# wkentaro/morefusion

Hardware: AMD Instinct MI355X
Metric: objects/sec (32^3 voxelize+3D-CNN+ICC refine) (higher is better)
Workload: dtype f32; 1 GPU; 1 scene(s) x 8 objects per GPU: singleview_3d Model.predict (ResNet18+PSPNet, 32^3 voxelize, occupancy 3D-CNN, heads; B=8) -> ICC joint refine 100 iters (BASELINE configs[1]+configs[2]); random weights, ICC starts from synthetic perturbed-GT poses; ICC(k) on a second HIP stream, event-ordered after network(k), beside network(k+1); objects_per_gpu=8, icc_iters=100, parallelism=scene-sharded x1, pose all_gather, stream_priority=none, backbone_memory_format=contiguous

## Files before the change

morefusion_amd/csrc/gemm_bf16.hip:

```cpp
#include <cstdlib>

#include "mf_common.h"

#include "gemm_bf16_nt.h"
#include "gemm_bf16_tn.h"
#include "gemm_bf16_aux.h"
#include "gemm_bf16_narrow.h"

namespace {

struct Knobs { int nt_big, nt_splitk, tn_pp, nt_half_max, pp_dbg; };
Knobs read_knobs() {
  auto num = [](const char *name, int unset) { const char *e = getenv(name); return e ? atoi(e) : unset; };
  Knobs k = {num("MF_NT_BIG", -1), num("MF_NT_SPLITK", 0), num("MF_TN_PP", 1), num("MF_NT_HALF_MAX", 255), 0};
#ifdef MF_PP_ABLATE
  k.pp_dbg = num("MF_PP_DBG", 0);
#endif
  return k;
}

constexpr int64_t kAnyWs = INT64_MAX;
struct NtShape { int mode; int64_t M; int N, K, groups; bool table; int64_t dgrad_rows; bool may_split; int64_t ws_bytes; };
struct NtPlan { int tile, S, dbg; };

NtPlan nt_plan(const NtShape &p, const Knobs &k) {
  const int64_t full = ((p.M + 127) / 128) * ((p.N + kBN - 1) / kBN) * p.groups;
  const int64_t big = ((p.M + kBigM - 1) / kBigM) * ((p.N + kBigN - 1) / kBigN) * p.groups;
  const bool dgrad = p.mode == kConvDgrad, can_big = !p.table && !(dgrad && (p.dgrad_rows & (kBigM - 1)));
  int S = 1;
  if (p.may_split && p.ws_bytes > 0 && can_big && p.N >= 192 && p.N % 8 == 0 && k.nt_big != 0) {
    const int T = (p.K + kBK - 1) / kBK;
    if (k.nt_splitk > 0) S = k.nt_splitk <= T ? k.nt_splitk : 1;
    else if (big >= 16 && big < 160)
      for (S = (int)(256 / big); S > 1 && T / S < 16;) --S;
    if (S > 1 && p.ws_bytes < S * p.M * p.N * 4) S = 1;
  }
  bool use_big = (big >= 224 && p.N >= 160 && can_big) || S > 1;
  if (k.nt_big == 2)
    use_big = can_big;
  else if (k.nt_big >= 0)
    use_big = use_big && k.nt_big == 1;
  if (use_big) return {kBigM, S, k.pp_dbg};
  const bool half = full <= k.nt_half_max && !dgrad;
  return {half ? 64 : 128, S, 0};
}

int64_t nt_workspace_bytes(int mode, int64_t M, int N, int K) {
  const NtPlan p = nt_plan({mode, M, N, K, 1, false, 0, true, kAnyWs}, read_knobs());
  return p.S > 1 ? p.S * M * N * 4 : 0;
}

int wgrad_split_model(int64_t tiles, int64_t ktiles, int64_t slab_bytes, int slots) {
  if (tiles <= 0 || ktiles <= 0) return 1;
  const double per_slab = slab_bytes / 3.0e6 > 0.05 ? slab_bytes / 3.0e6 : 0.05;
  int best = 1;
  double best_cost = 1e30;
  for (int S = 1; S <= 512; ++S) {
    if (S > 1 && ktiles / S < 8) break;
    const int64_t rounds = (tiles * S + slots - 1) / slots;
    const double cost = (double)rounds * (double)((ktiles + S - 1) / S + 8) + (S > 1 ? S * per_slab : 0.0);
    if (cost < best_cost) { best_cost = cost; best = S; }
  }
  return best;
}

struct TnShape { int Ni, Nj, ldc; int64_t ktiles; int groups; bool ranges, conv; int split; };
enum { kFinishNone = 0, kFinishPlain = 1, kFinishDeep = 2, kFinishConv = 3 };
struct TnPlan { bool pp; int split, finish; };

TnPlan tn_plan(const TnShape &p, const Knobs &k) {
  const int64_t tiles_pp = (int64_t)((p.Ni + 255) / 256) * ((p.Nj + 255) / 256) * p.groups;
  bool pp = k.tn_pp != 0 && k.nt_big != 0 && !p.ranges;
  if (pp && k.nt_big != 2)
    pp = p.Ni >= 192 && p.Nj >= 192 && p.ktiles >= 48 * (tiles_pp >= 256 ? 1 : (256 + tiles_pp - 1) / tiles_pp);
  const int64_t tiles = (int64_t)((p.Ni + 127) / 128) * ((p.Nj + 127) / 128) * p.groups, slab_bytes = 4ll * p.Ni * p.Nj * p.groups;
  const int split = p.split > 0 ? p.split : pp ? wgrad_split_model(tiles_pp, 2 * p.ktiles, slab_bytes, 256)
                                               : wgrad_split_model(tiles, p.ktiles, slab_bytes, 512);
  const int64_t per_slab = (int64_t)p.Ni * p.ldc * p.groups;
  int finish = split >= 32 && per_slab <= (1 << 16) ? kFinishDeep : kFinishPlain;
  if (p.conv && per_slab >= (1 << 20)) finish = kFinishConv;
  if (!p.conv && split == 1) finish = kFinishNone;
  return {pp, split, finish};
}

int g_nt_last_tile = 0;

template <int MODE, int MI>
int launch_nt_tile(const NtArgs &a, hipStream_t stream) {
  if (int e = mf::allow_big_lds((const void *)k_gemm_nt_bf16<MODE, MI>, nt_lds<MI>())) return e;
  const int64_t grid = (int64_t)((a.M + 64 * MI - 1) / (64 * MI)) * ((a.N + kBN - 1) / kBN) * a.groups;
  hipLaunchKernelGGL((k_gemm_nt_bf16<MODE, MI>), dim3((unsigned)grid), dim3(256), nt_lds<MI>(), stream, a);
  return 0;
}
template <int MODE>
int launch_nt(const NtArgs &a, const NtPlan &p, hipStream_t stream, const char *what) {
  g_nt_last_tile = p.tile;
  if (p.tile == kBigM) {
    const int64_t big = (int64_t)((a.M + kBigM - 1) / kBigM) * ((a.N + kBigN - 1) / kBigN) * a.groups;
    if (int e = mf::allow_big_lds((const void *)k_gemm_nt_bf16_pp<MODE>, nt_pp_lds())) return e;
    hipLaunchKernelGGL((k_gemm_nt_bf16_pp<MODE>), dim3((unsigned)(big * a.S)), dim3(512), nt_pp_lds(), stream, a);
    const dim3 finish((unsigned)(((int64_t)a.M * (a.N / 8) + 255) / 256));
    if (a.S > 1 && nt_split(MODE))
      hipLaunchKernelGGL(k_splitk_finish_conv2, finish, dim3(256), 0, stream, a);
    else if (a.S > 1)
      hipLaunchKernelGGL(k_splitk_finish, finish, dim3(256), 0, stream, (const float *)a.slab, a.bias, a.out,
                         (int64_t)a.M, a.N, a.S, a.ldo, a.relu, a.out_f32);
  } else if (int e = p.tile == 64 ? launch_nt_tile<MODE, 1>(a, stream) : launch_nt_tile<MODE, 2>(a, stream))
    return e;
  return mf::check_launch(what);
}

template <bool CONV>
int launch_tn(const TnArgs &a, const TnPlan &p, hipStream_t stream) {
  if (p.pp) {
    if (int e = mf::allow_big_lds((const void *)k_gemm_tn_bf16_pp<CONV>, 5 * kPpOp)) return e;
    const int64_t grid = (int64_t)((a.Ni + 255) / 256) * ((a.Nj + 255) / 256) * a.groups * a.S;
    hipLaunchKernelGGL(k_gemm_tn_bf16_pp<CONV>, dim3((unsigned)grid), dim3(512), 5 * kPpOp, stream, a);
    return 0;
  }
  if (int e = mf::allow_big_lds((const void *)k_gemm_tn_bf16<CONV>, kTnLds)) return e;
  const int64_t grid = (int64_t)((a.Ni + 127) / 128) * ((a.Nj + 127) / 128) * a.groups * a.S;
  hipLaunchKernelGGL(k_gemm_tn_bf16<CONV>, dim3((unsigned)grid), dim3(256), kTnLds, stream, a);
  return 0;
}

void launch_wgrad_finish(int finish, const TnArgs &a, float *dW, int w_cin, int keep, hipStream_t stream) {
  const int taps = a.conv ? a.ks * a.ks * a.ks : 0, cin = a.conv ? a.Cin : 0;
  const int64_t per_group = (int64_t)a.Ni * a.ldc, per_slab = per_group * a.groups;
  const int64_t pitch = a.conv ? (int64_t)w_cin * taps : a.ldc;
  if (finish == kFinishConv)
    hipLaunchKernelGGL(k_wgrad_finish_conv, dim3((keep + kPackTile - 1) / kPackTile, a.Ni), dim3(256), 0, stream,
                       (const float *)a.out, dW, per_slab, a.S, a.Cin, taps, w_cin, keep);
  else if (finish == kFinishDeep)
    hipLaunchKernelGGL(k_wgrad_finish_deep, dim3((unsigned)((per_slab + 3) / 4)), dim3(256), 0, stream,
                       (const float *)a.out, dW, per_slab, a.Nj, a.ldc, a.S, cin, a.c_gs, per_group, pitch, taps, keep);
  else if (finish == kFinishPlain)
    hipLaunchKernelGGL(k_wgrad_finish, dim3((unsigned)((per_slab + 255) / 256)), dim3(256), 0, stream,
                       (const float *)a.out, dW, per_slab, a.Nj, a.ldc, a.S, cin, a.c_gs, per_group, pitch, taps, keep);
}

constexpr int64_t kMaxBf16Elems = 1ll << 30;
int bad(const char *msg) {
  mf::set_last_error(hipErrorInvalidValue, msg);
  return -(int)hipErrorInvalidValue;
}

int ilog2_exact(int x) {
  int l = 0;
  while ((1 << l) < x) ++l;
  return (1 << l) == x ? l : -1;
}

struct Geom { int Do, olog, taps; };
int conv_geom(int B, int Cin, int Cout, int D, int ks, int stride, int pad, int dil, Geom *g) {
  const int span = dil * (ks - 1) + 1;
  if ((ks != 3 && ks != 4) || (stride != 1 && stride != 2) || dil < 1 || pad < 0 || D + 2 * pad < span)
    return bad("conv3d (bf16): kernel 3 or 4, stride 1 or 2");
  g->Do = (D + 2 * pad - span) / stride + 1;
  g->olog = ilog2_exact(g->Do);
  g->taps = ks * ks * ks;
  if (g->olog < 1 || Cin % 8 || Cout % 8 || (int64_t)B * D * D * D * Cin >= kMaxBf16Elems ||
      (int64_t)B * g->Do * g->Do * g->Do * Cout >= kMaxBf16Elems || (int64_t)Cout * g->taps * Cin >= kMaxBf16Elems)
    return bad("conv3d (bf16): output size a power of two, Cin % 8 == 0, Cout % 8 == 0, tensors < 2^30 elements (2^31 bytes)");
  return 0;
}

int conv2_geom(int B, int Cin, int Cout, int D, int ks, int stride, int pad, int dil, Geom *g) {
  const int span = dil * (ks - 1) + 1;
  if ((ks != 1 && ks != 3) || (stride != 1 && stride != 2) || dil < 1 || dil > 4 || pad < 0 || D + 2 * pad < span)
    return bad("conv2d_split: kernel 1 or 3, stride 1 or 2, dilation 1 .. 4");
  g->Do = (D + 2 * pad - span) / stride + 1;
  g->olog = ilog2_exact(g->Do);
  g->taps = ks * ks;
  if (g->olog < 0 || Cin % 8 || Cout % 8 || (int64_t)B * D * D * 2 * Cin >= kMaxBf16Elems ||
      (int64_t)B * g->Do * g->Do >= (1ll << 31) || (int64_t)Cout * g->taps * 3 * Cin >= kMaxBf16Elems)
    return bad("conv2d_split: output side a power of two, Cin % 8 == 0, Cout % 8 == 0, operands < 2^30 elements");
  return 0;
}

int split_out_check(const char *what, const float *bias, float *out32, int ldo32, void *outs, int ldos, int los, int N,
                    const float *res = nullptr, int ldr = 0) {
  if ((!out32 && !outs) || N % 8 || (out32 && (ldo32 < N || ldo32 % 8)) ||
      (outs && (ldos < N || ldos % 8 || los < N || los % 8 || ldos < los + N)) || (res && (ldr < N || ldr % 8)))
    return bad(what);
  if (((uintptr_t)bias | (uintptr_t)out32 | (uintptr_t)outs | (uintptr_t)res) & 15) return bad(what);
  return 0;
}

NtArgs nt_operands(const void *A, int lda, int64_t a_gs, const void *W, int ldw, int64_t w_gs, const float *bias,
                   int64_t b_gs, int64_t M, int N, int K, int groups, const int32_t *tile_group = nullptr) {
  NtArgs a = {};
  a.A = (const uint16_t *)A; a.W = (const uint16_t *)W; a.bias = bias;
  a.a_gs = a_gs; a.w_gs = w_gs; a.b_gs = b_gs;
  a.M = (int)M; a.N = N; a.K = K; a.lda = lda; a.ldw = ldw; a.groups = groups;
  a.tile_group = tile_group;
  return a;
}
void nt_conv_geom(NtArgs &a, int B, int D, const Geom &g, int Cin, int Cout, int ks, int stride, int pad, int dil) {
  a.B = B; a.D = D; a.Do = g.Do; a.olog = g.olog; a.Cin = Cin; a.Cout = Cout;
  a.ks = ks; a.stride = stride; a.pad = pad; a.dil = dil;
}
void nt_plain_out(NtArgs &a, void *out, int64_t o_gs, int ldo, int relu, int out_f32, int accumulate, const NtPlan &p,
                  void *ws = nullptr) {
  a.out = out; a.o_gs = o_gs; a.ldo = ldo; a.relu = relu; a.out_f32 = out_f32; a.accumulate = accumulate;
  a.S = p.S; a.slab = p.S > 1 ? (float *)ws : nullptr; a.dbg = p.dbg;
}
template <int MODE>
int launch_nt_split(NtArgs a, int xc, int act, float *out32, int ldo32, void *outs, int ldos, int los, void *ws,
                    int64_t ws_bytes, mfStream_t stream, const char *what, const float *res = nullptr, int ldr = 0,
                    const float *slope = nullptr) {
  const NtPlan p = nt_plan({MODE, a.M, a.N, a.K, 1, false, 0, true, ws ? ws_bytes : 0}, read_knobs());
  a.xc = xc; a.act = act; a.ldo32 = ldo32; a.ldos = ldos; a.los = los; a.out32 = out32; a.outs = (uint16_t *)outs;
  a.res = res; a.ldr = ldr; a.slope = slope;
  a.S = p.S; a.slab = p.S > 1 ? (float *)ws : nullptr; a.dbg = p.dbg;
  return launch_nt<MODE>(a, p, (hipStream_t)stream, what);
}

}

extern "C" int mf_gemm_bf16_nt_plan(int32_t mode, int64_t M, int32_t N, int32_t K, int32_t groups, int32_t table,
                                    int64_t dgrad_rows, int32_t may_split, int32_t have_ws, int32_t *tile, int32_t *S) {
  if (mode < kRows || mode > kRowsS || M <= 0 || N <= 0 || K <= 0 || groups <= 0 || !tile || !S)
    return bad("gemm_bf16_nt_plan: a mode 0 .. 5, a problem, somewhere to answer");
  const NtShape s = {mode, M, N, K, groups, table != 0, dgrad_rows, may_split != 0, have_ws ? kAnyWs : 0};
  const NtPlan p = nt_plan(s, read_knobs());
  *tile = p.tile; *S = p.S;
  return 0;
}

extern "C" int mf_gemm_bf16_tn_plan(int32_t Ni, int32_t Nj, int32_t ldc, int64_t rows, int32_t groups, int32_t ranges,
                                    int32_t conv, int32_t split, int32_t *form, int32_t *default_split, int32_t *finish) {
  if (Ni <= 0 || Nj <= 0 || ldc < Nj || rows < 0 || groups <= 0 || !form || !default_split || !finish)
    return bad("gemm_bf16_tn_plan: a problem with ldc >= Nj, somewhere to answer");
  const Knobs k = read_knobs();
  TnShape s = {Ni, Nj, ldc, (rows + 63) / 64, groups, ranges != 0, conv != 0, 0};
  *default_split = s.split = tn_plan(s, k).split;
  if (split > 0) s.split = split;
  const TnPlan p = tn_plan(s, k);
  *form = p.pp ? 256 : 128; *finish = p.finish;
  return 0;
}

extern "C" int mf_gemm_bf16_last_tile(void) { return g_nt_last_tile; }

extern "C" int mf_cast_rows_bf16(const float *src, int64_t src_ld, void *dst, int64_t dst_ld, int64_t rows,
                                 int32_t cols, mfStream_t stream_) {
  hipStream_t stream = (hipStream_t)stream_;
  if (rows <= 0) return 0;
  if (dst_ld % 8 || cols > dst_ld || src_ld < cols || ((uintptr_t)dst & 15)) return bad("cast_rows_bf16: dst_ld % 8 == 0, cols <= dst_ld");
  const int64_t n = rows * (dst_ld / 8);
  hipLaunchKernelGGL(k_cast_rows_bf16, dim3((unsigned)((n + 255) / 256)), dim3(256), 0, stream, src, src_ld,
                     (uint16_t *)dst, dst_ld, rows, cols);
  return mf::check_launch("mf_cast_rows_bf16");
}

extern "C" int mf_relu_mask_bf16(const void *y, const void *dy, const float *dy32, void *dz, int64_t n,
                                 mfStream_t stream_) {
  hipStream_t stream = (hipStream_t)stream_;
  if (n <= 0) return 0;
// ... 333 lines not shown
```

morefusion_amd/csrc/gemm_bf16_nt.h:

```cpp
#pragma once
#include "mf_common.h"

namespace {

using mf::mf_f32x16;

constexpr int kBN = 128, kBK = 64;
constexpr int kPitch = 144;
template <int MI> constexpr int nt_buf_bytes() { return (64 * MI + kBN) * kPitch; }
template <int MI> constexpr int nt_lds() {
  return 2 * nt_buf_bytes<MI>() > 64 * MI * (kBN + 4) * 4 ? 2 * nt_buf_bytes<MI>() : 64 * MI * (kBN + 4) * 4;
}

enum { kRows = 0, kConvFwd = 1, kConvDgrad = 2, kConv2Fwd = 3, kConvFwdS = 4, kRowsS = 5 };
constexpr bool nt_conv3(int mode) { return mode == kConvFwd || mode == kConvFwdS; }
constexpr bool nt_rows(int mode) { return mode == kRows || mode == kRowsS; }
constexpr bool nt_split(int mode) { return mode == kConv2Fwd || mode == kConvFwdS || mode == kRowsS; }

struct NtArgs {
  const uint16_t *A;
  const uint16_t *W;
  const float *bias;
  void *out;
  int64_t a_gs, w_gs, b_gs, o_gs;
  int M, N, K, lda, ldw, ldo, groups;
  int relu, out_f32, accumulate;
  const int32_t *tile_group;
  int B, D, Do, olog, Cin, Cout, ks, stride, pad, dil;
  int S;
  float *slab;
  int xc, act, ldr, ldo32, ldos, los;
  const float *res, *slope;
  float *out32;
  uint16_t *outs;
  int dbg;
};

__device__ __forceinline__ void conv2_store8(const NtArgs &a, int64_t m, int n, float *v) {
  if (a.bias) {
    const float4 b0 = *reinterpret_cast<const float4 *>(a.bias + n), b1 = *reinterpret_cast<const float4 *>(a.bias + n + 4);
    v[0] += b0.x; v[1] += b0.y; v[2] += b0.z; v[3] += b0.w; v[4] += b1.x; v[5] += b1.y; v[6] += b1.z; v[7] += b1.w;
  }
  if (a.res) {
    const float *r = a.res + m * a.ldr + n;
    const float4 r0 = *reinterpret_cast<const float4 *>(r), r1 = *reinterpret_cast<const float4 *>(r + 4);
    v[0] += r0.x; v[1] += r0.y; v[2] += r0.z; v[3] += r0.w; v[4] += r1.x; v[5] += r1.y; v[6] += r1.z; v[7] += r1.w;
  }
  if (a.act) {
    const float s = a.act == 2 ? *a.slope : 0.0f;
#pragma unroll
    for (int j = 0; j < 8; ++j) v[j] = v[j] > 0.0f ? v[j] : s * v[j];
  }
  if (a.out32) {
    float4 *o = reinterpret_cast<float4 *>(a.out32 + m * a.ldo32 + n);
    o[0] = make_float4(v[0], v[1], v[2], v[3]);
    o[1] = make_float4(v[4], v[5], v[6], v[7]);
  }
  if (a.outs) {
    uint32_t h[8], l[8];
#pragma unroll
    for (int j = 0; j < 8; ++j) {
      h[j] = mf::bf16_bits(v[j]);
      l[j] = mf::bf16_bits(v[j] - mf::bf16_lo(h[j]));
    }
    uint16_t *o = a.outs + m * a.ldos + n;
    *reinterpret_cast<uint4 *>(o) = make_uint4(h[0] | h[1] << 16, h[2] | h[3] << 16, h[4] | h[5] << 16, h[6] | h[7] << 16);
    *reinterpret_cast<uint4 *>(o + a.los) =
        make_uint4(l[0] | l[1] << 16, l[2] | l[3] << 16, l[4] | l[5] << 16, l[6] | l[7] << 16);
  }
}

template <int MODE, int MI>
__global__ __launch_bounds__(256, 2) void k_gemm_nt_bf16(NtArgs a) {
  MF_DYN_LDS(unsigned char, s_raw);
  constexpr int kBM = 64 * MI, kBuf = nt_buf_bytes<MI>();
  const int tiles_m = (a.M + kBM - 1) / kBM, tiles_n = (a.N + kBN - 1) / kBN;
  const int per_group = tiles_m * tiles_n;
  const int G = gridDim.x;
  int L = blockIdx.x;
  if ((G & 7) == 0) L = (blockIdx.x & 7) * (G >> 3) + (blockIdx.x >> 3);
  const int grp = L / per_group;
  const int rem = L - grp * per_group;
  const int m0 = (rem / tiles_n) * kBM, n0 = (rem % tiles_n) * kBN;
  const int T = (a.K + kBK - 1) / kBK;

  const int tid = threadIdx.x, wave = tid >> 6, lane = tid & 63;
  const int wm = wave & 1, wn = wave >> 1;
  const int lrow = lane & 31, lhalf = lane >> 5;
  const int chunk = tid & 7, r0 = tid >> 3;

  const int Do = a.Do, dol = a.olog;
  const uint16_t *A = a.A + grp * a.a_gs;
  const uint16_t *W = a.W + grp * a.w_gs;
  if (MODE == kRows && a.tile_group) {
    const int g = a.tile_group[m0 >> 6];
    if (g < 0) return;
    W += (int64_t)g * a.w_gs;
  }
  int cls = 0;
  if (MODE == kConvDgrad) {
    cls = (m0 >> (3 * dol)) & 7;
    W += (int64_t)cls * a.N * a.ldw;
  }
  int base[2 * MI], mask[2 * MI];
#pragma unroll
  for (int i = 0; i < 2 * MI; ++i) {
    const int m = m0 + r0 + 32 * i;
    const bool row_ok = m < a.M;
    const int mm = row_ok ? m : 0;
    int mk = row_ok ? 1 << 12 : 0;
    if (nt_rows(MODE)) {
      base[i] = mm * a.lda;
    } else if (MODE == kConv2Fwd) {
      const int b = mm >> (2 * dol), o = mm & ((1 << (2 * dol)) - 1);
      const int y0 = a.stride * (o >> dol) - a.pad, x0 = a.stride * (o & (Do - 1)) - a.pad;
      base[i] = ((b * a.D + y0) * a.D + x0) * a.xc;
#pragma unroll
      for (int k = 0; k < 4; ++k) {
        mk |= ((unsigned)(y0 + a.dil * k) < (unsigned)a.D ? 1 : 0) << k;
        mk |= ((unsigned)(x0 + a.dil * k) < (unsigned)a.D ? 1 : 0) << (4 + k);
      }
    } else if (nt_conv3(MODE)) {
      const int b = mm >> (3 * dol), o = mm & ((1 << (3 * dol)) - 1);
      const int ox = o >> (2 * dol), oy = (o >> dol) & (Do - 1), oz = o & (Do - 1);
      const int x0 = a.stride * ox - a.pad, y0 = a.stride * oy - a.pad, z0 = a.stride * oz - a.pad;
      base[i] = (((b * a.D + x0) * a.D + y0) * a.D + z0) * (MODE == kConvFwdS ? a.xc : a.Cin);
#pragma unroll
      for (int k = 0; k < 4; ++k) {
        mk |= ((unsigned)(x0 + a.dil * k) < (unsigned)a.D ? 1 : 0) << k;
        mk |= ((unsigned)(y0 + a.dil * k) < (unsigned)a.D ? 1 : 0) << (4 + k);
        mk |= ((unsigned)(z0 + a.dil * k) < (unsigned)a.D ? 1 : 0) << (8 + k);
      }
    } else {
      const int h = mm & ((1 << (3 * dol)) - 1), b = mm >> (3 * dol + 3);
      const int hx = h >> (2 * dol), hy = (h >> dol) & (Do - 1), hz = h & (Do - 1);
      const int ux = hx + (cls & 1), uy = hy + ((cls >> 1) & 1), uz = hz + ((cls >> 2) & 1);
      base[i] = (((b * Do + ux) * Do + uy) * Do + uz) * a.Cout;
#pragma unroll
      for (int s = 0; s < 2; ++s) {
        mk |= ((unsigned)(ux - s) < (unsigned)Do ? 1 : 0) << s;
        mk |= ((unsigned)(uy - s) < (unsigned)Do ? 1 : 0) << (4 + s);
        mk |= ((unsigned)(uz - s) < (unsigned)Do ? 1 : 0) << (8 + s);
      }
    }
    mask[i] = mk;
  }
  uint32_t wrow[4];
#pragma unroll
  for (int i = 0; i < 4; ++i) {
    const int n = n0 + r0 + 32 * i;
    wrow[i] = 2u * (uint32_t)((int64_t)(n < a.N ? n : 0) * a.ldw);
  }

  mf_f32x16 acc[MI][2];
#pragma unroll
  for (int i = 0; i < MI; ++i)
#pragma unroll
    for (int j = 0; j < 2; ++j)
#pragma unroll
      for (int e = 0; e < 16; ++e) acc[i][j][e] = 0.0f;

  uint4 ra0P, ra1P, ra2P = make_uint4(0u, 0u, 0u, 0u), ra3P = ra2P, rb0P, rb1P, rb2P, rb3P;
  int kg = 8 * chunk, tc = 0, tx = 0, ty = 0, tz = 0;
  if (nt_conv3(MODE)) {
    const int tap = kg / a.Cin;
    tc = kg - tap * a.Cin;
    const int kxy = tap / a.ks;
    tz = tap - kxy * a.ks; tx = kxy / a.ks; ty = kxy - tx * a.ks;
  } else if (MODE == kConv2Fwd) {
    const int tap = kg / a.Cin;
    tc = kg - tap * a.Cin;
    tx = tap / a.ks; ty = tap - tx * a.ks;
  } else if (MODE == kConvDgrad) {
    tx = kg / a.Cout;
    tc = kg - tx * a.Cout;
  }
  const mf::BufRsrc Ars = mf::make_rsrc(A), Wrs = mf::make_rsrc(W);
#define MF_NT_LOAD_A(S, i_, reg_)                                                                     \
  reg_ = mf::buf_load16(Ars, (mask[i_] & bits_) == bits_ ? 2u * (uint32_t)(base[i_] + off_) : mf::kBufMasked);
#define MF_NT_LOAD_B(S, i_, reg_) reg_ = mf::buf_load16(Wrs, wrow[i_] + kofs_);
#define MF_NT_FETCH(S)                                                                                \
  {                                                                                                   \
    const bool kin_ = kg + 8 <= a.K;                                                                  \
    const uint32_t kofs_ = kin_ ? 2u * (uint32_t)kg : 0u;                                             \
    int off_ = MODE == kRowsS && kg >= a.xc ? kg - a.xc : kg, bits_ = 1 << 12;                        \
    if (nt_conv3(MODE)) {                                                                             \
      off_ = ((tx * a.D + ty) * a.D + tz) * a.dil * (MODE == kConvFwdS ? a.xc : a.Cin) +              \
             (MODE == kConvFwdS && tc >= a.xc ? tc - a.xc : tc);                                      \
      bits_ = tx < a.ks ? (1 << tx) | (16 << ty) | (256 << tz) | (1 << 12) : 1 << 13;                 \
    } else if (MODE == kConv2Fwd) {                                                                   \
      off_ = (tx * a.D + ty) * a.dil * a.xc + (tc >= a.xc ? tc - a.xc : tc);                          \
      bits_ = tx < a.ks ? (1 << tx) | (16 << ty) | (1 << 12) : 1 << 13;                               \
    } else if (MODE == kConvDgrad) {                                                                  \
      const int sx = tx & 1, sy = (tx >> 1) & 1, sz = tx >> 2;                                        \
      off_ = tc - ((sx * Do + sy) * Do + sz) * a.Cout;                                                \
      bits_ = (1 << sx) | (16 << sy) | (256 << sz) | (1 << 12);                                       \
    }                                                                                                 \
    if (!kin_) bits_ = 1 << 13;                                              \
    MF_NT_LOAD_A(S, 0, ra0##S) MF_NT_LOAD_A(S, 1, ra1##S)                                             \
    if constexpr (MI == 2) { MF_NT_LOAD_A(S, 2 * MI - 2, ra2##S) MF_NT_LOAD_A(S, 2 * MI - 1, ra3##S) } \
    MF_NT_LOAD_B(S, 0, rb0##S) MF_NT_LOAD_B(S, 1, rb1##S) MF_NT_LOAD_B(S, 2, rb2##S) MF_NT_LOAD_B(S, 3, rb3##S) \
    kg += kBK;                                                                                        \
    if (nt_conv3(MODE)) {                                                                             \
      tc += kBK;                                                                                      \
      while (tc >= a.Cin) {                                                                           \
        tc -= a.Cin;                                                                                  \
        if (++tz == a.ks) { tz = 0; if (++ty == a.ks) { ty = 0; ++tx; } }                             \
      }                                                                                               \
    } else if (MODE == kConv2Fwd) {                                                                   \
      tc += kBK;                                                                                      \
      while (tc >= a.Cin) {                                                                           \
        tc -= a.Cin;                                                                                  \
        if (++ty == a.ks) { ty = 0; ++tx; }                                                           \
      }                                                                                               \
    } else if (MODE == kConvDgrad) {                                                                  \
      tc += kBK;                                                                                      \
      while (tc >= a.Cout) { tc -= a.Cout; ++tx; }                                                    \
    }                                                                                                 \
  }
#define MF_NT_STASH(S, buf_)                                                                          \
  {                                                                                                   \
    MF_HOLD(ra0##S); MF_HOLD(ra1##S); MF_HOLD(rb0##S); MF_HOLD(rb1##S); MF_HOLD(rb2##S); MF_HOLD(rb3##S); \
    if constexpr (MI == 2) { MF_HOLD(ra2##S); MF_HOLD(ra3##S); }                                      \
    unsigned char *As_ = s_raw + (buf_) * kBuf + r0 * kPitch + 16 * chunk;                            \
    unsigned char *Bs_ = As_ + kBM * kPitch;                                                          \
    *reinterpret_cast<uint4 *>(As_) = ra0##S; *reinterpret_cast<uint4 *>(As_ + 32 * kPitch) = ra1##S; \
    if constexpr (MI == 2) {                                                                          \
      *reinterpret_cast<uint4 *>(As_ + 64 * kPitch) = ra2##S; *reinterpret_cast<uint4 *>(As_ + 96 * kPitch) = ra3##S; \
    }                                                                                                 \
    *reinterpret_cast<uint4 *>(Bs_) = rb0##S; *reinterpret_cast<uint4 *>(Bs_ + 32 * kPitch) = rb1##S; \
    *reinterpret_cast<uint4 *>(Bs_ + 64 * kPitch) = rb2##S; *reinterpret_cast<uint4 *>(Bs_ + 96 * kPitch) = rb3##S; \
  }
#ifndef MF_NT_PIPE
#define MF_NT_PIPE 1
#endif
#define MF_NT_FRAGS(set_, s_, NJ_)                                                                    \
  {                                                                                                   \
    fa[set_][0] = *reinterpret_cast<const uint4 *>(As + 32 * (s_));                                   \
    if constexpr (MI == 2) fa[set_][1] = *reinterpret_cast<const uint4 *>(As + 32 * kPitch + 32 * (s_)); \
    fb[set_][0] = *reinterpret_cast<const uint4 *>(Bs + 32 * (s_));                                   \
    if constexpr (NJ_ == 2) fb[set_][1] = *reinterpret_cast<const uint4 *>(Bs + 32 * kPitch + 32 * (s_)); \
  }
#define MF_NT_COMPUTE(buf_, NJ_)                                                                      \
  {                                                                                                   \
    asm volatile("" ::: "memory");                                                                    \
    __builtin_amdgcn_sched_barrier(0);                                                                \
    const unsigned char *As = s_raw + (buf_) * kBuf + (wm * 32 * MI + lrow) * kPitch + 16 * lhalf;    \
    const unsigned char *Bs = s_raw + (buf_) * kBuf + (kBM + wn * 64 + lrow) * kPitch + 16 * lhalf;   \
    if constexpr (MF_NT_PIPE) {                                                                       \
      uint4 fa[2][2], fb[2][2];                                                                       \
      MF_NT_FRAGS(0, 0, NJ_)                                                                          \
      __builtin_amdgcn_sched_group_barrier(0x100, MI + NJ_, 0);                                       \
      _Pragma("unroll") for (int s = 0; s < 4; ++s) {                                                 \
        const int c = s & 1;                                                                          \
        if (s < 3) MF_NT_FRAGS(c ^ 1, s + 1, NJ_)                                                     \
        _Pragma("unroll") for (int mi = 0; mi < MI; ++mi) {                                           \
          acc[mi][0] = mf::mfma_bf16_32x32x16(fa[c][mi], fb[c][0], acc[mi][0]);                       \
          if constexpr (NJ_ == 2) acc[mi][1] = mf::mfma_bf16_32x32x16(fa[c][mi], fb[c][1], acc[mi][1]); \
        }                                                                                             \
        if (s < 3) __builtin_amdgcn_sched_group_barrier(0x100, MI + NJ_, 0);                          \
        __builtin_amdgcn_sched_group_barrier(0x008, MI * NJ_, 0);                                     \
      }                                                                                               \
    } else {                                                                                          \
      _Pragma("unroll") for (int s = 0; s < 4; ++s) {                                                 \
        const uint4 a0 = *reinterpret_cast<const uint4 *>(As + 32 * s);                               \
        const uint4 b0 = *reinterpret_cast<const uint4 *>(Bs + 32 * s);                               \
        acc[0][0] = mf::mfma_bf16_32x32x16(a0, b0, acc[0][0]);                                        \
        if constexpr (NJ_ == 2) {                                                                     \
          const uint4 b1 = *reinterpret_cast<const uint4 *>(Bs + 32 * kPitch + 32 * s);               \
          acc[0][1] = mf::mfma_bf16_32x32x16(a0, b1, acc[0][1]);                                      \
          if constexpr (MI == 2) {                                                                    \
            const uint4 a1 = *reinterpret_cast<const uint4 *>(As + 32 * kPitch + 32 * s);             \
            acc[MI - 1][0] = mf::mfma_bf16_32x32x16(a1, b0, acc[MI - 1][0]);                          \
            acc[MI - 1][1] = mf::mfma_bf16_32x32x16(a1, b1, acc[MI - 1][1]);                          \
          }                                                                                           \
        } else if constexpr (MI == 2) {                                                               \
          const uint4 a1 = *reinterpret_cast<const uint4 *>(As + 32 * kPitch + 32 * s);               \
          acc[MI - 1][0] = mf::mfma_bf16_32x32x16(a1, b0, acc[MI - 1][0]);                            \
        }                                                                                             \
      }                                                                                               \
    }                                                                                                 \
    __builtin_amdgcn_sched_barrier(0);                                                                \
  }
  const int ncols = a.N - (n0 + wn * 64);
  MF_NT_FETCH(P);
  MF_NT_STASH(P, 0);
  __syncthreads();
  for (int t = 0; t < T; ++t) {
    MF_NT_FETCH(P);
    if (ncols > 32) MF_NT_COMPUTE(t & 1, 2) else if (ncols > 0) MF_NT_COMPUTE(t & 1, 1)
    MF_NT_STASH(P, (t + 1) & 1);
    __syncthreads();
  }
#undef MF_NT_FRAGS
#undef MF_NT_COMPUTE
#undef MF_NT_STASH
#undef MF_NT_FETCH
#undef MF_NT_LOAD_B
#undef MF_NT_LOAD_A

  constexpr int kEp = kBN + 4;
  float *s_out = reinterpret_cast<float *>(s_raw);
  const float *bias = a.bias && !nt_split(MODE) ? a.bias + grp * a.b_gs : nullptr;
#pragma unroll
  for (int mi = 0; mi < MI; ++mi)
#pragma unroll
    for (int ni = 0; ni < 2; ++ni) {
      const int nl = wn * 64 + ni * 32 + lrow;
      const float bn = (bias && n0 + nl < a.N) ? bias[n0 + nl] : 0.0f;
#pragma unroll
      for (int e = 0; e < 16; ++e) {
        const int ml = wm * 32 * MI + mi * 32 + (e & 3) + 8 * (e >> 2) + 4 * lhalf;
        float v = acc[mi][ni][e] + bn;
        if (a.relu && !nt_split(MODE)) v = v > 0.0f ? v : 0.0f;
        s_out[ml * kEp + nl] = v;
      }
    }
  __syncthreads();
  for (int i = tid; i < kBM * (kBN / 8); i += 256) {
    const int ml = i / (kBN / 8), c8 = i - ml * (kBN / 8);
    const int m = m0 + ml, n = n0 + 8 * c8;
    if (m >= a.M || n >= a.N) continue;
    int64_t orow = m;
    if (MODE == kConvDgrad) {
      const int h = m & ((1 << (3 * dol)) - 1), p = (m >> (3 * dol)) & 7, b = m >> (3 * dol + 3);
      const int x = 2 * (h >> (2 * dol)) + (p & 1), y = 2 * ((h >> dol) & (Do - 1)) + ((p >> 1) & 1),
                z = 2 * (h & (Do - 1)) + (p >> 2);
      orow = (((int64_t)b * a.D + x) * a.D + y) * a.D + z;
    }
    const float4 v0 = *reinterpret_cast<const float4 *>(s_out + ml * kEp + 8 * c8);
    const float4 v1 = *reinterpret_cast<const float4 *>(s_out + ml * kEp + 8 * c8 + 4);
    float v[8] = {v0.x, v0.y, v0.z, v0.w, v1.x, v1.y, v1.z, v1.w};
    if (nt_split(MODE)) {
      conv2_store8(a, m, n, v);
      continue;
    }
    const int nv = a.N - n < 8 ? a.N - n : 8;
    if (a.out_f32) {
      float *o = reinterpret_cast<float *>(a.out) + grp * a.o_gs + orow * a.ldo + n;
      if (nv == 8 && (a.ldo & 3) == 0 && ((uintptr_t)o & 15) == 0) {
        float4 *o4 = reinterpret_cast<float4 *>(o);
        if (a.accumulate) {
          const float4 p0 = o4[0], p1 = o4[1];
          v[0] += p0.x; v[1] += p0.y; v[2] += p0.z; v[3] += p0.w;
          v[4] += p1.x; v[5] += p1.y; v[6] += p1.z; v[7] += p1.w;
        }
        o4[0] = make_float4(v[0], v[1], v[2], v[3]);
        o4[1] = make_float4(v[4], v[5], v[6], v[7]);
      } else {
        for (int j = 0; j < nv; ++j) o[j] = a.accumulate ? o[j] + v[j] : v[j];
      }
    } else {
      uint16_t *o = reinterpret_cast<uint16_t *>(a.out) + grp * a.o_gs + orow * a.ldo + n;
      if (nv == 8 && (a.ldo & 7) == 0 && ((uintptr_t)o & 15) == 0) {
        *reinterpret_cast<uint4 *>(o) = make_uint4(mf::pack_bf16x2(v[0], v[1]), mf::pack_bf16x2(v[2], v[3]),
                                                   mf::pack_bf16x2(v[4], v[5]), mf::pack_bf16x2(v[6], v[7]));
      } else {
        for (int j = 0; j < nv; ++j) o[j] = (uint16_t)mf::bf16_bits(v[j]);
      }
    }
  }
}

constexpr int kBigM = 256, kBigN = 256;

constexpr int kPpOp = 256 * 128;
constexpr int kPpW0 = 3 * kPpOp;
constexpr int nt_pp_lds() { return 5 * kPpOp; }

template <int MODE>
__global__ __launch_bounds__(512, 2) void k_gemm_nt_bf16_pp(NtArgs a) {
  MF_DYN_LDS(unsigned char, s_raw);
  constexpr int kBM = kBigM, kBNb = kBigN;
  const int tiles_m = (a.M + kBM - 1) / kBM, tiles_n = (a.N + kBNb - 1) / kBNb;
  const int per_group = tiles_m * tiles_n;
  const int G = gridDim.x;
  int L = blockIdx.x;
  if ((G & 7) == 0) L = (blockIdx.x & 7) * (G >> 3) + (blockIdx.x >> 3);
  const int split = L / (per_group * a.groups);
  L -= split * per_group * a.groups;
  const int grp = L / per_group;
  const int rem = L - grp * per_group;
  const int m0 = (rem / tiles_n) * kBM, n0 = (rem % tiles_n) * kBNb;
  const int Tall = (a.K + kBK - 1) / kBK, Tper = (Tall + a.S - 1) / a.S;
  const int t0 = split * Tper;
  const int T = max(0, min(Tall, t0 + Tper) - t0);

  const int tid = threadIdx.x, lane = tid & 63;
  const int wave = mf::wave_uniform(tid >> 6);
  const int wm = wave >> 2, wn = wave & 3;
  const int lrow = lane & 31, lhalf = lane >> 5;
  const int r0 = tid >> 3;
  const int chunk = (tid & 7) ^ ((r0 >> 1) & 7);

  const int Do = a.Do, dol = a.olog;
  const uint16_t *A = a.A + grp * a.a_gs;
  const uint16_t *W = a.W + grp * a.w_gs;
  int cls = 0;
  if (MODE == kConvDgrad) {
    cls = (m0 >> (3 * dol)) & 7;
    W += (int64_t)cls * a.N * a.ldw;
  }
  int base[4], mask[4];
#pragma unroll
  for (int i = 0; i < 4; ++i) {
    const int m = m0 + r0 + 64 * i;
    const bool row_ok = m < a.M;
    const int mm = row_ok ? m : 0;
    int mk = row_ok ? 1 << 12 : 0;
    if (nt_rows(MODE)) {
      base[i] = mm * a.lda;
    } else if (MODE == kConv2Fwd) {
      const int b = mm >> (2 * dol), o = mm & ((1 << (2 * dol)) - 1);
      const int y0 = a.stride * (o >> dol) - a.pad, x0 = a.stride * (o & (Do - 1)) - a.pad;
      base[i] = ((b * a.D + y0) * a.D + x0) * a.xc;
#pragma unroll
      for (int k = 0; k < 4; ++k) {
        mk |= ((unsigned)(y0 + a.dil * k) < (unsigned)a.D ? 1 : 0) << k;
        mk |= ((unsigned)(x0 + a.dil * k) < (unsigned)a.D ? 1 : 0) << (4 + k);
      }
    } else if (nt_conv3(MODE)) {
      const int b = mm >> (3 * dol), o = mm & ((1 << (3 * dol)) - 1);
      const int ox = o >> (2 * dol), oy = (o >> dol) & (Do - 1), oz = o & (Do - 1);
      const int x0 = a.stride * ox - a.pad, y0 = a.stride * oy - a.pad, z0 = a.stride * oz - a.pad;
      base[i] = (((b * a.D + x0) * a.D + y0) * a.D + z0) * (MODE == kConvFwdS ? a.xc : a.Cin);
#pragma unroll
      for (int k = 0; k < 4; ++k) {
        mk |= ((unsigned)(x0 + a.dil * k) < (unsigned)a.D ? 1 : 0) << k;
        mk |= ((unsigned)(y0 + a.dil * k) < (unsigned)a.D ? 1 : 0) << (4 + k);
        mk |= ((unsigned)(z0 + a.dil * k) < (unsigned)a.D ? 1 : 0) << (8 + k);
      }
    } else {
      const int h = mm & ((1 << (3 * dol)) - 1), b = mm >> (3 * dol + 3);
      const int hx = h >> (2 * dol), hy = (h >> dol) & (Do - 1), hz = h & (Do - 1);
      const int ux = hx + (cls & 1), uy = hy + ((cls >> 1) & 1), uz = hz + ((cls >> 2) & 1);
      base[i] = (((b * Do + ux) * Do + uy) * Do + uz) * a.Cout;
#pragma unroll
      for (int s = 0; s < 2; ++s) {
        mk |= ((unsigned)(ux - s) < (unsigned)Do ? 1 : 0) << s;
        mk |= ((unsigned)(uy - s) < (unsigned)Do ? 1 : 0) << (4 + s);
        mk |= ((unsigned)(uz - s) < (unsigned)Do ? 1 : 0) << (8 + s);
      }
    }
    mask[i] = mk;
  }
  uint32_t wrow[4];
#pragma unroll
  for (int i = 0; i < 4; ++i) {
    const int n = n0 + r0 + 64 * i;
    wrow[i] = 2u * (uint32_t)((int64_t)(n < a.N ? n : 0) * a.ldw);
  }

  mf_f32x16 acc[4][2];
#pragma unroll
  for (int i = 0; i < 4; ++i)
#pragma unroll
    for (int j = 0; j < 2; ++j)
#pragma unroll
      for (int e = 0; e < 16; ++e) acc[i][j][e] = 0.0f;

  int kg = 8 * chunk + kBK * t0, tc = 0, tx = 0, ty = 0, tz = 0, kgw = kg;
  if (nt_conv3(MODE)) {
    const int tap = kg / a.Cin;
    tc = kg - tap * a.Cin;
    const int kxy = tap / a.ks;
    tz = tap - kxy * a.ks; tx = kxy / a.ks; ty = kxy - tx * a.ks;
  } else if (MODE == kConv2Fwd) {
    const int tap = kg / a.Cin;
    tc = kg - tap * a.Cin;
    tx = tap / a.ks; ty = tap - tx * a.ks;
  } else if (MODE == kConvDgrad) {
    tx = kg / a.Cout;
    tc = kg - tx * a.Cout;
  }
  const mf::BufRsrc Ars = mf::make_rsrc(A), Wrs = mf::make_rsrc(W);
  unsigned char *const dma0 = s_raw + 8 * wave * 128;
#define MF_PP_REQ_A(sa_, i0_, i1_)                                                                    \
  {                                                                                                   \
    const bool kin_ = kg + 8 <= a.K;                                                                  \
    int off_ = MODE == kRowsS && kg >= a.xc ? kg - a.xc : kg, bits_ = 1 << 12;                        \
    if (nt_conv3(MODE)) {                                                                             \
      off_ = ((tx * a.D + ty) * a.D + tz) * a.dil * (MODE == kConvFwdS ? a.xc : a.Cin) +              \
             (MODE == kConvFwdS && tc >= a.xc ? tc - a.xc : tc);                                      \
      bits_ = tx < a.ks ? (1 << tx) | (16 << ty) | (256 << tz) | (1 << 12) : 1 << 13;                 \
    } else if (MODE == kConv2Fwd) {                                                                   \
// ... 190 lines not shown
```

Before: 2028 objects/sec.

## Add split-K path for small-tile conv2 NT GEMMs with slab finish

Adds a split-K mode to the small/medium-tile NT GEMM kernel for 2D-conv forward shapes with narrow N (at most 128), chosen by a simple cost model that weighs per-split K work against slab traffic. Each split writes fp32 partials to a workspace slab, and the existing conv2 finish kernel reduces them and applies the epilogue. The aim is to fill the GPU when few output tiles exist but K is long, such as the backbone's low-channel convolutions. The cost is extra slab writes and reads plus one more kernel launch per GEMM.

```diff
diff --git a/morefusion_amd/csrc/gemm_bf16.hip b/morefusion_amd/csrc/gemm_bf16.hip
--- a/morefusion_amd/csrc/gemm_bf16.hip
+++ b/morefusion_amd/csrc/gemm_bf16.hip
@@ -9,10 +9,11 @@
 
 namespace {
 
-struct Knobs { int nt_big, nt_splitk, tn_pp, nt_half_max, pp_dbg; };
+struct Knobs { int nt_big, nt_splitk, tn_pp, nt_half_max, pp_dbg, nt_small_splitk; };
 Knobs read_knobs() {
   auto num = [](const char *name, int unset) { const char *e = getenv(name); return e ? atoi(e) : unset; };
-  Knobs k = {num("MF_NT_BIG", -1), num("MF_NT_SPLITK", 0), num("MF_TN_PP", 1), num("MF_NT_HALF_MAX", 255), 0};
+  Knobs k = {num("MF_NT_BIG", -1), num("MF_NT_SPLITK", 0), num("MF_TN_PP", 1), num("MF_NT_HALF_MAX", 255), 0,
+             num("MF_NT_SMALL_SPLITK", -1)};
 #ifdef MF_PP_ABLATE
   k.pp_dbg = num("MF_PP_DBG", 0);
 #endif
@@ -22,6 +23,17 @@
 constexpr int64_t kAnyWs = INT64_MAX;
 struct NtShape { int mode; int64_t M; int N, K, groups; bool table; int64_t dgrad_rows; bool may_split; int64_t ws_bytes; };
 struct NtPlan { int tile, S, dbg; };
+
+constexpr int kSmallSplitMinT = 8;
+int small_splitk_model(int64_t tiles, int T, int64_t slab_bytes) {
+  int best = 1;
+  double best_cost = 0.5 * T - 2.0;
+  for (int S = 2; tiles * S <= 256 && T / S >= kSmallSplitMinT; ++S) {
+    const double cost = 0.5 * ((T + S - 1) / S) + 3.0 + 0.35e-6 * (double)S * (double)slab_bytes;
+    if (cost < best_cost) { best_cost = cost; best = S; }
+  }
+  return best;
+}
 
 NtPlan nt_plan(const NtShape &p, const Knobs &k) {
   const int64_t full = ((p.M + 127) / 128) * ((p.N + kBN - 1) / kBN) * p.groups;
@@ -42,6 +54,14 @@
     use_big = use_big && k.nt_big == 1;
   if (use_big) return {kBigM, S, k.pp_dbg};
   const bool half = full <= k.nt_half_max && !dgrad;
+  if (S == 1 && p.mode == kConv2Fwd && p.may_split && p.ws_bytes > 0 && p.N % 8 == 0 && k.nt_small_splitk != 0) {
+    const int T = (p.K + kBK - 1) / kBK;
+    const int64_t tiles = half ? ((p.M + 63) / 64) * ((p.N + kBN - 1) / kBN) : full;
+    if (k.nt_small_splitk > 0) S = k.nt_small_splitk <= T ? k.nt_small_splitk : 1;
+    else if (p.N <= kBN)
+      S = small_splitk_model(tiles, T, p.M * p.N * 4);
+    if (S > 1 && p.ws_bytes < S * p.M * p.N * 4) S = 1;
+  }
   return {half ? 64 : 128, S, 0};
 }
 
@@ -85,11 +105,11 @@
 
 int g_nt_last_tile = 0;
 
-template <int MODE, int MI>
+template <int MODE, int MI, bool KSPLIT = false>
 int launch_nt_tile(const NtArgs &a, hipStream_t stream) {
-  if (int e = mf::allow_big_lds((const void *)k_gemm_nt_bf16<MODE, MI>, nt_lds<MI>())) return e;
-  const int64_t grid = (int64_t)((a.M + 64 * MI - 1) / (64 * MI)) * ((a.N + kBN - 1) / kBN) * a.groups;
-  hipLaunchKernelGGL((k_gemm_nt_bf16<MODE, MI>), dim3((unsigned)grid), dim3(256), nt_lds<MI>(), stream, a);
+  if (int e = mf::allow_big_lds((const void *)k_gemm_nt_bf16<MODE, MI, KSPLIT>, nt_lds<MI>())) return e;
+  const int64_t grid = (int64_t)((a.M + 64 * MI - 1) / (64 * MI)) * ((a.N + kBN - 1) / kBN) * a.groups * (KSPLIT ? a.S : 1);
+  hipLaunchKernelGGL((k_gemm_nt_bf16<MODE, MI, KSPLIT>), dim3((unsigned)grid), dim3(256), nt_lds<MI>(), stream, a);
   return 0;
 }
 template <int MODE>
@@ -105,6 +125,12 @@
     else if (a.S > 1)
       hipLaunchKernelGGL(k_splitk_finish, finish, dim3(256), 0, stream, (const float *)a.slab, a.bias, a.out,
                          (int64_t)a.M, a.N, a.S, a.ldo, a.relu, a.out_f32);
+  } else if (a.S > 1 && MODE == kConv2Fwd) {
+    if constexpr (MODE == kConv2Fwd) {
+      if (int e = p.tile == 64 ? launch_nt_tile<MODE, 1, true>(a, stream) : launch_nt_tile<MODE, 2, true>(a, stream)) return e;
+      hipLaunchKernelGGL(k_splitk_finish_conv2, dim3((unsigned)(((int64_t)a.M * (a.N / 8) + 255) / 256)), dim3(256), 0,
+                         stream, a);
+    }
   } else if (int e = p.tile == 64 ? launch_nt_tile<MODE, 1>(a, stream) : launch_nt_tile<MODE, 2>(a, stream))
     return e;
   return mf::check_launch(what);
diff --git a/morefusion_amd/csrc/gemm_bf16_nt.h b/morefusion_amd/csrc/gemm_bf16_nt.h
--- a/morefusion_amd/csrc/gemm_bf16_nt.h
+++ b/morefusion_amd/csrc/gemm_bf16_nt.h
@@ -70,7 +70,7 @@
   }
 }
 
-template <int MODE, int MI>
+template <int MODE, int MI, bool KSPLIT = false>
 __global__ __launch_bounds__(256, 2) void k_gemm_nt_bf16(NtArgs a) {
   MF_DYN_LDS(unsigned char, s_raw);
   constexpr int kBM = 64 * MI, kBuf = nt_buf_bytes<MI>();
@@ -79,10 +79,18 @@
   const int G = gridDim.x;
   int L = blockIdx.x;
   if ((G & 7) == 0) L = (blockIdx.x & 7) * (G >> 3) + (blockIdx.x >> 3);
+  int split = 0;
+  if constexpr (KSPLIT) {
+    const int tile = L / a.S;
+    split = L - tile * a.S;
+    L = tile;
+  }
   const int grp = L / per_group;
   const int rem = L - grp * per_group;
   const int m0 = (rem / tiles_n) * kBM, n0 = (rem % tiles_n) * kBN;
-  const int T = (a.K + kBK - 1) / kBK;
+  const int Tall = (a.K + kBK - 1) / kBK;
+  const int t0 = KSPLIT ? split * Tall / a.S : 0;
+  const int T = KSPLIT ? (split + 1) * Tall / a.S - t0 : Tall;
 
   const int tid = threadIdx.x, wave = tid >> 6, lane = tid & 63;
   const int wm = wave & 1, wn = wave >> 1;
@@ -161,7 +169,7 @@
       for (int e = 0; e < 16; ++e) acc[i][j][e] = 0.0f;
 
   uint4 ra0P, ra1P, ra2P = make_uint4(0u, 0u, 0u, 0u), ra3P = ra2P, rb0P, rb1P, rb2P, rb3P;
-  int kg = 8 * chunk, tc = 0, tx = 0, ty = 0, tz = 0;
+  int kg = 8 * chunk + kBK * t0, tc = 0, tx = 0, ty = 0, tz = 0;
   if (nt_conv3(MODE)) {
     const int tap = kg / a.Cin;
     tc = kg - tap * a.Cin;
@@ -331,6 +339,12 @@
     const float4 v0 = *reinterpret_cast<const float4 *>(s_out + ml * kEp + 8 * c8);
     const float4 v1 = *reinterpret_cast<const float4 *>(s_out + ml * kEp + 8 * c8 + 4);
     float v[8] = {v0.x, v0.y, v0.z, v0.w, v1.x, v1.y, v1.z, v1.w};
+    if constexpr (KSPLIT) {
+      float4 *o = reinterpret_cast<float4 *>(a.slab + ((int64_t)split * a.M + m) * a.N + n);
+      o[0] = v0;
+      o[1] = v1;
+      continue;
+    }
     if (nt_split(MODE)) {
       conv2_store8(a, m, n, v);
       continue;
```

Result: no change. 2026 objects/sec (-0.1%).
